# mikkleini/slam.net

Measured on AMD Instinct MI355X. Metric: candidate-pose distance evals/sec on 2048^2 map, 1080-ray scan, 1/2/4/8 GPU, higher is better.
Workload: dtype f32 transform + u16 gather / integer sum

## Files before the change

slam.net_amd/csrc/distance.hip:

```cpp
#include "cs_internal.h"
#include "det_trig.h"
#include <stdlib.h>
#include <algorithm>

#define K1_THREADS 256

__device__ static inline void k1_coords(const float4 q, const float2 p, float &fx, float &fy)
{
    fx = q.x + q.z * p.x;  fx = fx - q.w * p.y;
    fy = q.y + q.w * p.x;  fy = fy + q.z * p.y;
}

template <bool SAFE>
__device__ static inline void k1_gather_global(const uint16_t *__restrict__ map, int S, const float4 q, const float2 p,
                                               uint32_t &sum, uint32_t &cnt)
{
    float fx, fy;
    k1_coords(q, p, fx, fy);
    int ix, iy;
    if (SAFE) { ix = sh_f2i(fx); iy = sh_f2i(fy); }
    else      { ix = (int)fx;    iy = (int)fy; }
    const bool ok = ((unsigned)ix < (unsigned)S) & ((unsigned)iy < (unsigned)S);
    uint32_t v = 0;
    if (ok) v = map[(size_t)iy * S + ix];
// ... 187 lines not shown
__device__ static inline unsigned k1_tile_addr(int ix, int iy, int pitch2, int kofs)
{
    unsigned t, a;
    asm("v_lshl_add_u32 %0, %1, 1, %2" : "=v"(t) : "v"(ix), "s"(kofs));
    asm("v_mad_u32_u24 %0, %1, %2, %3" : "=v"(a) : "v"(iy), "s"(pitch2), "v"(t));
    return a;
}
__device__ static inline float k1_den(int v) { return __uint_as_float(v < 0 ? (0x80000000u | (unsigned)(-v)) : (unsigned)v); }
__device__ static inline unsigned k1_tile_addr_d(float fx, float fy, float two_d, float pitch2_d, float c_d)
{
    const float g = fmaf(truncf(fy), pitch2_d, fmaf(truncf(fx), two_d, c_d));
    return __float_as_uint(g);
}
typedef __attribute__((address_space(3))) const uint16_t k1_lds_u16;
__device__ static inline uint32_t k1_lds_load(unsigned addr) { return *(k1_lds_u16 *)(size_t)addr; }
typedef __attribute__((address_space(3))) const float k1_lds_f;
__device__ static inline float2 k1_point_lds(unsigned lds_addr)
{
    k1_lds_f *p = (k1_lds_f *)(size_t)lds_addr;
    return make_float2(p[0], p[1]);
}

typedef float k1_f32x4a8 __attribute__((ext_vector_type(4), aligned(8)));
__device__ static inline float4 k1_points2_lds(unsigned lds_addr)
{
    const k1_f32x4a8 v = *(__attribute__((address_space(3))) const k1_f32x4a8 *)(size_t)lds_addr;
    return make_float4(v.x, v.y, v.z, v.w);
}

__device__ static inline void k1_ray_box(const float *b, const float2 p, int &x0, int &y0, int &x1, int &y1)
{
    const float cx0 = b[4] * p.x, cx1 = b[5] * p.x, sy0 = b[6] * p.y, sy1 = b[7] * p.y;
    const float sx0 = b[6] * p.x, sx1 = b[7] * p.x, cy0 = b[4] * p.y, cy1 = b[5] * p.y;
    float xlo = b[0] + fminf(cx0, cx1);  xlo = xlo - fmaxf(sy0, sy1);
    float xhi = b[1] + fmaxf(cx0, cx1);  xhi = xhi - fminf(sy0, sy1);
    float ylo = b[2] + fminf(sx0, sx1);  ylo = ylo + fminf(cy0, cy1);
    float yhi = b[3] + fmaxf(sx0, sx1);  yhi = yhi + fmaxf(cy0, cy1);
    x0 = (int)xlo; x1 = (int)xhi; y0 = (int)ylo; y1 = (int)yhi;
}

__device__ static inline int k1_div(int a, int b)
{
    int q = (int)((float)a * __builtin_amdgcn_rcpf((float)b));
    const int r = a - q * b;
    if (r < 0) q--; else if (r >= b) q++;
    return q;
}

template <int CTRL, int ROWS> __device__ static inline int k1_dpp(int v) { return __builtin_amdgcn_update_dpp(v, v, CTRL, ROWS, 0xf, false); }
template <bool MAX> __device__ static inline int k1_wave_red(int x)
{
#define K1_MM(a, b) (MAX ? max(a, b) : min(a, b))
    x = K1_MM(x, (k1_dpp<0xB1, 0xf>(x)));
    x = K1_MM(x, (k1_dpp<0x4E, 0xf>(x)));
    x = K1_MM(x, (k1_dpp<0x124, 0xf>(x)));
    x = K1_MM(x, (k1_dpp<0x128, 0xf>(x)));
    x = K1_MM(x, (k1_dpp<0x142, 0xa>(x)));
    x = K1_MM(x, (k1_dpp<0x143, 0xc>(x)));
#undef K1_MM
    return x;
}
template <bool MAX> __device__ static inline float k1_wave_redf(float x)
{
#define K1_MM(a, b) (MAX ? fmaxf(a, b) : fminf(a, b))
    x = K1_MM(x, __int_as_float(k1_dpp<0xB1, 0xf>(__float_as_int(x))));
    x = K1_MM(x, __int_as_float(k1_dpp<0x4E, 0xf>(__float_as_int(x))));
    x = K1_MM(x, __int_as_float(k1_dpp<0x124, 0xf>(__float_as_int(x))));
    x = K1_MM(x, __int_as_float(k1_dpp<0x128, 0xf>(__float_as_int(x))));
    x = K1_MM(x, __int_as_float(k1_dpp<0x142, 0xa>(__float_as_int(x))));
    x = K1_MM(x, __int_as_float(k1_dpp<0x143, 0xc>(__float_as_int(x))));
#undef K1_MM
    return x;
}

struct k1_wg_t { int g, nc, nbp, bp, rlo, rhi, chunk; };
__device__ __forceinline__ k1_wg_t k1_wg_decode(const k1_args &a, const int bid)
{
    int g, chunk, nc, nbp = 1;
    if ((int)bid < a.n_tab_wgs) {
        const unsigned pw = ((const unsigned *)a.wg_pos)[bid >> 2];
        const int p = (int)((pw >> ((bid & 3u) * 8u)) & 0xffu);
        const k1_args::tab_rec rec = a.tab[p];
        nc = rec.nc;
        chunk = bid - (int)rec.first;
        g = rec.group;
        nbp = rec.nbp;
    } else {
        const int b = bid - a.n_tab_wgs;
        nc = a.uni_nc;
        chunk = b / (unsigned)a.uni_ng;
        g = a.uni_g0 + (b - chunk * a.uni_ng);
    }
    const int rc = chunk / nbp, bp = chunk - rc * nbp, nrc = nc / nbp;
    int rlo, rhi;
#define K1_CUT(i) ((int)((((const unsigned *)a.cut)[(i) >> 1] >> (((i) & 1) * 16)) & 0xffffu))
    if (a.uni_cut && (int)bid >= a.n_tab_wgs) {
        rlo = K1_CUT(chunk); rhi = K1_CUT(chunk + 1);
    } else if (a.tab_cut && (int)bid < a.n_tab_wgs) {
        const int i0 = a.tab_cut + (int)bid;
        rlo = K1_CUT(i0);
        rhi = rc + 1 < nrc ? K1_CUT(i0 + nbp) : a.n_rays;
    } else
#undef K1_CUT
    if (a.n_rays <= 46340) {
        rlo = (int)(((unsigned)rc * (unsigned)a.n_rays) / (unsigned)nrc); rhi = (int)(((unsigned)(rc + 1) * (unsigned)a.n_rays) / (unsigned)nrc);
    } else { rlo = (int)(((long long)rc * a.n_rays) / nrc); rhi = (int)(((long long)(rc + 1) * a.n_rays) / nrc); }
    k1_wg_t W; W.g = g; W.nc = nc; W.nbp = nbp; W.bp = bp; W.rlo = rlo; W.rhi = rhi; W.chunk = chunk;
    return W;
}

__device__ __forceinline__ void k1_bounds_from_jitter(const k1_args &a, const float gb[6], float *bnd, const int lane)
{
    const float scale = a.scale;
    const float pxl = (a.bx + gb[0]) * scale + 0.5f, pxh = (a.bx + gb[1]) * scale + 0.5f;
    const float pyl = (a.by + gb[2]) * scale + 0.5f, pyh = (a.by + gb[3]) * scale + 0.5f;
    const float tlf = a.bth + gb[4], thf = a.bth + gb[5];
    const double n2 = rint((double)tlf * 0.15915494309189535) * 6.283185307179586;
    const float rl = (float)((double)tlf - n2), rh = (float)((double)thf - n2);
    const float as = scale, pad = as * 1.0e-4f;
    const float cl = __cosf(rl) * as, ch = __cosf(rh) * as, sl = __sinf(rl) * as, sh = __sinf(rh) * as;
    float clo = fminf(cl, ch) - pad, chi = fmaxf(cl, ch) + pad, slo = fminf(sl, sh) - pad, shi = fmaxf(sl, sh) + pad;
    const bool all = !(rh - rl < 6.2f);
    {
        const int k_lo = (int)ceilf((rl - 1.0e-3f) * 0.636619772f), span = (int)floorf((rh + 1.0e-3f) * 0.636619772f) - k_lo;
        if (all || ((0 - k_lo) & 3) <= span) chi = as + pad;
        if (all || ((1 - k_lo) & 3) <= span) shi = as + pad;
        if (all || ((2 - k_lo) & 3) <= span) clo = -as - pad;
        if (all || ((3 - k_lo) & 3) <= span) slo = -as - pad;
    }
    const float4 qlo = make_float4(pxl, pyl, 0.f, 0.f), qhi = make_float4(pxh, pyh, 0.f, 0.f);
    if (lane == 0) {
        *(float4 *)&bnd[0] = make_float4(qlo.x, qhi.x, qlo.y, qhi.y);
        *(float4 *)&bnd[4] = make_float4(clo, chi, slo, shi);
    }
}

#ifndef K1_DMA0
#define K1_DMA0 0
#endif
#ifndef K1_EXP
#define K1_EXP 0
#endif
typedef unsigned int k1_u32x4 __attribute__((ext_vector_type(4)));

#ifndef K1_VGPR_CAP
#define K1_VGPR_CAP __attribute__((amdgpu_num_vgpr(104)))
#endif
template <int MODE, bool VERIFY, int CPL, int GROUP, bool LAT = false>
__global__ void __launch_bounds__(GROUP / CPL, GROUP / CPL / 64 / 2) K1_VGPR_CAP
k1_search_tiled(const k1_args a)
{
    constexpr int LANES = GROUP / CPL, NW = LANES / 64, PF = 65536 / (LANES * 16);
    constexpr int RU = (K1_MAXR + LANES - 1) / LANES;
    extern __shared__ __attribute__((aligned(16))) char smem[];
    const unsigned smem_lds = (unsigned)(size_t)(__attribute__((address_space(3))) char *)smem;
    __shared__ __attribute__((aligned(16))) int stepbuf[K1_MAXSTEPS * 8];
    __shared__ __attribute__((aligned(16))) float2 cpts[K1_MAXR + 4];
    __shared__ int2 pieces[K1_MAXP];
    __shared__ __attribute__((aligned(16))) float wred[NW][8];
    __shared__ __attribute__((aligned(16))) float bnd[8];
    __shared__ unsigned long long wkey[NW];
    __shared__ unsigned wfin[NW];
    __shared__ int s_nsteps;
    __shared__ int s_plan_ok;
    const unsigned cpts_lds = (unsigned)(size_t)(__attribute__((address_space(3))) char *)cpts;

    const uint16_t *__restrict__ map = a.map;
    const int S = a.S, count = a.count;
    const int t = threadIdx.x, lane = t & 63;
    int zv;
    asm volatile("v_mov_b32 %0, 0" : "=v"(zv));
    const int wv = __builtin_amdgcn_readfirstlane(t >> 6);
    const k1_wg_t W = k1_wg_decode(a, (int)blockIdx.x);
    const int g = W.g, nc = W.nc, nbp = W.nbp;
    if (a.ring_reset && blockIdx.x == 0 && t == 0)
        __hip_atomic_store(a.ring_reset, ~0ull, __ATOMIC_RELAXED, __HIP_MEMORY_SCOPE_AGENT);
    if (a.started && blockIdx.x == 0 && t == 0)
        __hip_atomic_store(a.started, a.launch_no, __ATOMIC_RELAXED, __HIP_MEMORY_SCOPE_SYSTEM);
    K1_STAMP(0)
#ifdef K1_TIMES
    if (t == 0 && blockIdx.x < 4096) { for (int k = 0; k < 8; k++) g_k1_sub[blockIdx.x * 8 + k] = 0; }
    if (t == 0 && blockIdx.x < 4096) { for (int k = 10; k < 16; k++) g_k1_times[blockIdx.x * 16 + k] = 0; g_k1_times[blockIdx.x * 16 + 14] = (unsigned long long)g; g_k1_times[blockIdx.x * 16 + 15] = (unsigned long long)nc; }
    if (lane == 0 && blockIdx.x < 4096) g_k1_wstart[blockIdx.x * 16 + (wv & 15)] = wall_clock64();
    if (t == 0 && blockIdx.x < 4096) {
        unsigned hw, xcc;
        asm volatile("s_getreg_b32 %0, hwreg(HW_REG_HW_ID)" : "=s"(hw));
        asm volatile("s_getreg_b32 %0, hwreg(HW_REG_XCC_ID)" : "=s"(xcc));
        g_k1_wstart[blockIdx.x * 16 + 15] = ((unsigned long long)(xcc & 15u) << 16) | ((hw >> 8) & 0xffu);
    }
#endif
    const int bp = W.bp, rlo = W.rlo, rhi = W.rhi;
    const int nrays = rhi - rlo;
    if (a.scan_flag) {
        uint32_t v = 0;
        if (wv == 0) {
            int spins = 0;
            for (;;) {
                v = __hip_atomic_load(a.scan_flag, __ATOMIC_RELAXED, __HIP_MEMORY_SCOPE_SYSTEM);
                if ((v & 0x7fffffffu) == a.scan_seq) break;
                if (++spins > (1 << 23)) { if (t == 0) atomicAdd(a.verify, 1u); v = 0x80000000u; break; }
                __builtin_amdgcn_s_sleep(32);
            }
            if (blockIdx.x == 0 && t == 0) { ((uint32_t *)a.scan_flag)[8] = (uint32_t)spins; ((uint32_t *)a.scan_flag)[9] += (uint32_t)spins; }
            if (lane == 0) s_plan_ok = (int)v;
        }
        __syncthreads();
        v = (uint32_t)s_plan_ok;
        __syncthreads();
        if (__builtin_amdgcn_readfirstlane(v) & 0x80000000u) return;
    }
    const int blk_first = a.ray_blk[rlo + zv].z;
    const int blk_last_v = a.ray_blk[rhi - 1 + zv].z;

    const bool pre = MODE == 1 && a.grp_bounds != nullptr;
    float gb[6];
    if (pre) {
#pragma unroll
        for (int k = 0; k < 6; k++) gb[k] = a.grp_bounds[8 * (size_t)g + k];
    }
    const bool planned = MODE == 1 && !LAT && pre && a.plan_rec != nullptr;
    uint2 prw = make_uint2(0u, 0u);
    if (planned && wv == 0) prw = a.plan_rec[(size_t)blockIdx.x * (K1_PLAN_REC_WORDS / 2) + lane];
    float4 q[CPL];
    float c3[CPL][3];
#pragma unroll
    for (int k = 0; k < CPL; k++) {
        const int j = g * GROUP + k * LANES + t;
        const int jc = j < count ? j : count - 1;
        if (MODE == 0) q[k] = a.pxcs[jc];
        else { c3[k][0] = a.src3[3 * jc]; c3[k][1] = a.src3[3 * jc + 1]; c3[k][2] = a.src3[3 * jc + 2]; }
    }
    int4 rinfo[RU];
    float2 rpt[RU];
#pragma unroll
    for (int u = 0; u < RU; u++) {
        const int i = u * LANES + t;
        const int r = rlo + (i < nrays ? i : 0);
        rinfo[u] = make_int4(0, 0, 0, 0); rpt[u] = make_float2(0.f, 0.f);
        if (i < nrays) { rinfo[u] = a.ray_blk[r]; rpt[u] = a.pts[r]; }
    }
    if (t == 0) { s_nsteps = 0; s_plan_ok = 0; *(unsigned *)(smem + K1_ZERO_OFS) = 0u; }
    if (MODE != 0 && !pre) {
#pragma unroll
        for (int k = 0; k < CPL; k++) q[k] = k1_candidate<MODE == 0 ? 1 : MODE, true>(c3[k], a.bx, a.by, a.bth, a.scale);
    }
#pragma unroll
    for (int u = 0; u < RU; u++) {
        const int i = u * LANES + t;
        if (i < nrays) {
            cpts[i] = rpt[u];
            if (i == 0 || rinfo[u].x == rlo + i)
                pieces[rinfo[u].z - blk_first] = make_int2(i, (rinfo[u].y < rhi ? rinfo[u].y : rhi) - (rlo + i));
        }
    }
    bool have_plan = false;
    if (planned) {
        if (wv == 0) {
            const bool okl = ((lane & 3) != 3 || prw.y == a.plan_seq) && (lane != 0 || prw.x == a.plan_seq);
            const int ns = __builtin_amdgcn_readfirstlane((int)prw.y);
            const bool ok = __builtin_amdgcn_ballot_w64(okl) == ~0ull && ns >= 0 && ns <= K1_PLAN_STEPS;
            if (lane >= 4) *(int2 *)&stepbuf[2 * lane - 8] = make_int2((int)prw.x, (int)prw.y);
            if (lane == 0 && ok) { s_plan_ok = 1; s_nsteps = ns; }
        }
        __syncthreads();
        have_plan = __builtin_amdgcn_readfirstlane(s_plan_ok) != 0;
        if (VERIFY && t == 0) atomicAdd(a.verify + (have_plan ? 5 : 6), 1u);
    }
    K1_STAMP(1)
    if (!have_plan) {
    if (pre) {
        if (wv == 0) {
            k1_bounds_from_jitter(a, gb, bnd, lane);
        }
        __syncthreads();
        K1_STAMP(2)
    } else
    {
        float lo[4] = { q[0].x, q[0].y, q[0].z, q[0].w }, hi[4] = { q[0].x, q[0].y, q[0].z, q[0].w };
#pragma unroll
        for (int k = 1; k < CPL; k++) {
            lo[0] = fminf(lo[0], q[k].x); hi[0] = fmaxf(hi[0], q[k].x); lo[1] = fminf(lo[1], q[k].y); hi[1] = fmaxf(hi[1], q[k].y);
            lo[2] = fminf(lo[2], q[k].z); hi[2] = fmaxf(hi[2], q[k].z); lo[3] = fminf(lo[3], q[k].w); hi[3] = fmaxf(hi[3], q[k].w);
        }
        const float m0 = k1_wave_redf<false>(lo[0]), m1 = k1_wave_redf<true>(hi[0]);
        const float m2 = k1_wave_redf<false>(lo[1]), m3 = k1_wave_redf<true>(hi[1]);
        const float m4 = k1_wave_redf<false>(lo[2]), m5 = k1_wave_redf<true>(hi[2]);
        const float m6 = k1_wave_redf<false>(lo[3]), m7 = k1_wave_redf<true>(hi[3]);
        if (lane == 63) {
            *(float4 *)&wred[wv][0] = make_float4(m0, m1, m2, m3);
            *(float4 *)&wred[wv][4] = make_float4(m4, m5, m6, m7);
        }
        __syncthreads();
        K1_STAMP(2)
        if (t < 8) {
            float v[NW];
#pragma unroll
            for (int w = 0; w < NW; w++) v[w] = wred[w][t];
            float x = v[0];
#pragma unroll
            for (int w = 1; w < NW; w++) x = (t & 1) ? fmaxf(x, v[w]) : fminf(x, v[w]);
            bnd[t] = x;
        }
        __syncthreads();
    }
    K1_STAMP(3)
    const int npieces = __builtin_amdgcn_readfirstlane(blk_last_v - blk_first + 1);
#define K1_PIECE_STAMP K1_STAMP(4)
#define K1_STEP_SLOT(i) (i)
#define K1_PIECE_RAY(i) (i)
#include "k1_pieces.inc"
#undef K1_PIECE_RAY
#undef K1_STEP_SLOT
#undef K1_PIECE_STAMP
    __syncthreads();
    }
#ifdef K1_TIMES
    else if (t == 0 && blockIdx.x < 4096) { const unsigned long long now_ = wall_clock64(); for (int k = 2; k <= 4; k++) g_k1_times[blockIdx.x * 16 + k] = now_; }
#endif
    const int nsteps = s_nsteps;
    K1_STAMP(5)

    uint32_t sum[CPL], cnt[CPL];
#pragma unroll
    for (int k = 0; k < CPL; k++) { sum[k] = 0; cnt[k] = 0; }
    if (LAT && !(MODE != 0 && a.grp_bounds != nullptr)) {
#pragma unroll
        for (int k = 1; k < CPL; k++)
            if (g * GROUP + k * LANES + t < count && (__float_as_uint(q[k].z) != __float_as_uint(q[0].z) || __float_as_uint(q[k].w) != __float_as_uint(q[0].w)))
                atomicAdd(a.verify, 1u);
    }
    uint32_t cnt_all = 0;
    if (nsteps > 0) {
        k1_u32x4 R[PF];
        int dst[PF];
#define K1_PREFETCH(step, enable)                                                                   \
        {                                                                                           \
             \
             \
             \
            const int4 pa_ = *(const int4 *)&stepbuf[(step) * 8];                                   \
            const int shift_ = __builtin_amdgcn_readfirstlane(stepbuf[(step) * 8 + 4]);             \
            const int w8_ = __builtin_amdgcn_readfirstlane(pa_.z), h_ = (enable) ? __builtin_amdgcn_readfirstlane(pa_.w) : 0; \
            const int rpi = 64 >> shift_;                          \
            const int srow = lane >> shift_, scol = lane & ((1 << shift_) - 1);                     \
            const bool colok = scol < (w8_ >> 3);                                                   \
            const int cc = colok ? scol : 0;                                                        \
            const unsigned S2_ = (unsigned)S * 2u;                                                  \
            const unsigned gofs = ((unsigned)__builtin_amdgcn_readfirstlane(pa_.y) * (unsigned)S + (unsigned)__builtin_amdgcn_readfirstlane(pa_.x)) * 2u; \
            const int pitchb = w8_ << 1;                                                            \
            const int row0 = wv * rpi + srow, rstep = NW * rpi;                                     \
            unsigned vofs = gofs + (unsigned)row0 * S2_ + ((unsigned)cc << 4);                      \
            int ldsd = K1_TILE_OFS + (cc << 4) + row0 * pitchb;                                     \
            const unsigned vstep = (unsigned)rstep * S2_;                                           \
            const int lstep = rstep * pitchb;                                                       \
            _Pragma("unroll") for (int k_ = 0; k_ < PF; k_++) {                                     \
                const bool live = colok & (row0 + k_ * rstep < h_);                                 \
                if (live && K1_EXP != 3) R[k_] = *(const k1_u32x4 *)((const char *)map + vofs);    \
                dst[k_] = live ? ldsd : -1;                                                         \
                vofs += vstep; ldsd += lstep;                                                       \
            }                                                                                       \
        }
#if K1_DMA0
        {
            const int4 pa_ = *(const int4 *)&stepbuf[0];
            const int w8_ = __builtin_amdgcn_readfirstlane(pa_.z), h_ = __builtin_amdgcn_readfirstlane(pa_.w);
            const int ncols = w8_ >> 3, nunits = ncols * h_;
            const unsigned S2_ = (unsigned)S * 2u;
            const unsigned gofs = ((unsigned)__builtin_amdgcn_readfirstlane(pa_.y) * (unsigned)S + (unsigned)__builtin_amdgcn_readfirstlane(pa_.x)) * 2u;
            const float rn = 1.0f / (float)ncols;
#pragma unroll
            for (int k_ = 0; k_ < PF; k_++) {
                const int e0 = (k_ * NW + wv) * 64;
                if (e0 < nunits && K1_EXP != 3) {
                    const int e = e0 + lane;
                    const int row = (int)(((float)e + 0.5f) * rn);
                    const int col = e - row * ncols;
                    if (e < nunits)
                        __builtin_amdgcn_global_load_lds((const __attribute__((address_space(1))) void *)((const char *)map + (gofs + (unsigned)row * S2_ + ((unsigned)col << 4))),
                                                         (__attribute__((address_space(3))) void *)(smem + K1_TILE_OFS + (e0 << 4)), 16, 0, 0);
                }
            }
#pragma unroll
            for (int k_ = 0; k_ < PF; k_++) dst[k_] = -1;
        }
#else
        K1_PREFETCH(0, true)
#endif
        if (MODE != 0 && pre) {
            {
#pragma unroll
            for (int k = 0; k < CPL; k++) { if (K1_EXP == 1) q[k] = make_float4(a.bx * a.scale + c3[k][0], a.by * a.scale + c3[k][1], a.scale, c3[k][2]); else q[k] = k1_candidate<MODE == 0 ? 1 : MODE, true>(c3[k], a.bx, a.by, a.bth, a.scale); }
            }
            if (LAT) {
#pragma unroll
                for (int k = 1; k < CPL; k++)
                    if (g * GROUP + k * LANES + t < count && (__float_as_uint(q[k].z) != __float_as_uint(q[0].z) || __float_as_uint(q[k].w) != __float_as_uint(q[0].w)))
                        atomicAdd(a.verify, 1u);
            }
        }
#ifdef K1_TIMES
        const unsigned long long sclk0 = clock64();
#endif
        for (int s = 0; s < nsteps; s++) {
#ifdef K1_TIMES
            const unsigned long long ts0 = wall_clock64();
#endif
            if (K1_DMA0 && s == 0) asm volatile("s_waitcnt vmcnt(0)" ::: "memory");
            else {
            __syncthreads();
#pragma unroll
            for (int k = 0; k < PF; k++) asm volatile("" : "+v"(R[k]));
#pragma unroll
            for (int k = 0; k < PF; k++) if (dst[k] >= 0 && K1_EXP != 3) *(k1_u32x4 *)(smem + dst[k]) = R[k];
            }
            __syncthreads();
            if (s == 0) K1_STAMP(6)
#ifdef K1_TIMES
            const unsigned long long ts1 = wall_clock64();
            if (s > 0) K1_SUB(0, ts1 - ts0)
#endif
            const int4 ca = *(const int4 *)&stepbuf[s * 8], cb = *(const int4 *)&stepbuf[s * 8 + 4];
            {
                const int sn = s + 1 < nsteps ? s + 1 : s;
                K1_PREFETCH(sn, s + 1 < nsteps)
            }
#ifdef K1_TIMES
            const unsigned long long ts2 = wall_clock64();
            K1_SUB(1, ts2 - ts1) K1_SUB(3, 1ull)
#endif
            const int kind = __builtin_amdgcn_readfirstlane(cb.y);
            const int nr = __builtin_amdgcn_readfirstlane(cb.z) >> 16;
#ifdef K1_TIMES
            if (t == 0 && blockIdx.x < 4096) g_k1_times[blockIdx.x * 16 + 10 + kind] += (unsigned long long)nr;
            if (t == 0 && blockIdx.x < 4096 && s < 3)
                g_k1_sub[blockIdx.x * 8 + 5 + s] = (unsigned long long)kind | ((unsigned long long)__builtin_amdgcn_readfirstlane(ca.z) << 4) | ((unsigned long long)__builtin_amdgcn_readfirstlane(ca.w) << 16) | ((unsigned long long)nr << 32);
#endif
            const unsigned pbase = cpts_lds + (unsigned)zv + (unsigned)(__builtin_amdgcn_readfirstlane(cb.z) & 0xffff) * 8u;
            const int x0a = __builtin_amdgcn_readfirstlane(ca.x), y0 = __builtin_amdgcn_readfirstlane(ca.y);
            const int w8 = __builtin_amdgcn_readfirstlane(ca.z), h = __builtin_amdgcn_readfirstlane(ca.w);
            const int pitch2 = w8 << 1;
            const int kofs = (int)smem_lds + K1_TILE_OFS - ((y0 * w8 + x0a) << 1);
            const unsigned zaddr = smem_lds + K1_ZERO_OFS + (unsigned)zv;
            const bool daddr = !a.noden && (unsigned)S * (unsigned)pitch2 + 2u * (unsigned)S + (1u << 18) < (1u << 23);
            float two_v, p2d_v, cd_v;
            {
                const float two_s = k1_den(2), p2d_s = k1_den(pitch2), cd_s = k1_den(kofs);
                asm volatile("v_mov_b32 %0, %1" : "=v"(two_v) : "s"(two_s));
                asm volatile("v_mov_b32 %0, %1" : "=v"(p2d_v) : "s"(p2d_s));
                asm volatile("v_mov_b32 %0, %1" : "=v"(cd_v) : "s"(cd_s));
            }
            if (K1_EXP == 2 || K1_EXP == 3) { sum[0] += (uint32_t)nr; continue; }
            if (kind != K1_KIND_GLOBAL) {
                const bool checked = kind == K1_KIND_BAND;
                uint32_t va[CPL], vb[CPL];
                int r = 0;
                float4 pn = k1_points2_lds(pbase);
                float2 pa_n = make_float2(pn.x, pn.y), pb_n = make_float2(pn.z, pn.w);
#pragma unroll
                for (int k = 0; k < CPL; k++) { va[k] = k1_lds_load(zaddr); vb[k] = k1_lds_load(zaddr); }
                __builtin_amdgcn_sched_barrier(0);
                if (!checked && daddr) {
#define K1_DPAIR(P, NEXTREAD)                                                                       \
                    {                                                                               \
                        unsigned ada[CPL], adb[CPL];                                                \
                        float cxa_ = 0.f, sya_ = 0.f, sxa_ = 0.f, cya_ = 0.f, cxb_ = 0.f, syb_ = 0.f, sxb_ = 0.f, cyb_ = 0.f; \
                        if (LAT) {                                                                  \
                            cxa_ = q[0].z * (P).x; sya_ = q[0].w * (P).y; sxa_ = q[0].w * (P).x; cya_ = q[0].z * (P).y; \
                            cxb_ = q[0].z * (P).z; syb_ = q[0].w * (P).w; sxb_ = q[0].w * (P).z; cyb_ = q[0].z * (P).w; \
                        }                                                                           \
                        _Pragma("unroll") for (int k = 0; k < CPL; k++) {                           \
                            float fxa, fya, fxb, fyb;                                               \
                            if (LAT) {                                                              \
                                fxa = q[k].x + cxa_; fxa = fxa - sya_; fya = q[k].y + sxa_; fya = fya + cya_; \
                                fxb = q[k].x + cxb_; fxb = fxb - syb_; fyb = q[k].y + sxb_; fyb = fyb + cyb_; \
                            } else {                                                                \
                                k1_coords(q[k], make_float2((P).x, (P).y), fxa, fya);               \
                                k1_coords(q[k], make_float2((P).z, (P).w), fxb, fyb);               \
                            }                                                                       \
                            ada[k] = k1_tile_addr_d(fxa, fya, two_v, p2d_v, cd_v);                  \
                            adb[k] = k1_tile_addr_d(fxb, fyb, two_v, p2d_v, cd_v);                  \
                            if (VERIFY) {                                                           \
                                const int ixa = (int)fxa, iya = (int)fya, ixb = (int)fxb, iyb = (int)fyb; \
                                if (ixa < x0a || ixa >= x0a + w8 || iya < y0 || iya >= y0 + h ||    \
                                    ixb < x0a || ixb >= x0a + w8 || iyb < y0 || iyb >= y0 + h) atomicAdd(a.verify, 1u); \
                                else if (ada[k] != k1_tile_addr(ixa, iya, pitch2, kofs) || adb[k] != k1_tile_addr(ixb, iyb, pitch2, kofs) || \
                                         map[(size_t)iya * S + ixa] != *(const uint16_t *)(smem + (ada[k] - smem_lds)) || \
                                         map[(size_t)iyb * S + ixb] != *(const uint16_t *)(smem + (adb[k] - smem_lds))) \
                                    atomicAdd(a.verify, 1u);                \
                            }                                                                       \
                        }                                                                           \
                        __builtin_amdgcn_sched_barrier(0);                                          \
                        NEXTREAD;      \
                        _Pragma("unroll") for (int k = 0; k < CPL; k++) sum[k] += va[k] + vb[k];    \
                        _Pragma("unroll") for (int k = 0; k < CPL; k++) { va[k] = k1_lds_load(ada[k]); vb[k] = k1_lds_load(adb[k]); } \
                        __builtin_amdgcn_sched_barrier(0);                                          \
                    }
                    for (; r + 3 < nr; r += 4) {
                        const float4 p0 = pn;
                        float4 p1;
                        K1_DPAIR(p0, p1 = k1_points2_lds(pbase + r * 8 + 16))
                        K1_DPAIR(p1, pn = k1_points2_lds(pbase + r * 8 + 32))
                    }
                    if (r + 1 < nr) {
                        const float4 p0 = pn;
                        K1_DPAIR(p0, pn = k1_points2_lds(pbase + r * 8 + 16))
                        r += 2;
                    }
#undef K1_DPAIR
                    pa_n = make_float2(pn.x, pn.y);
                    cnt_all += (uint32_t)nr;
                } else if (!checked) {
                    for (; r + 1 < nr; r += 2) {
                        const float2 pa = pa_n, pb = pb_n;
                        pa_n = k1_point_lds(pbase + r * 8 + 16); pb_n = k1_point_lds(pbase + r * 8 + 24);
                        unsigned ada[CPL], adb[CPL];
#pragma unroll
                        for (int k = 0; k < CPL; k++) {
                            float fxa, fya, fxb, fyb;
                            k1_coords(q[k], pa, fxa, fya);
                            k1_coords(q[k], pb, fxb, fyb);
                            const int ixa = (int)fxa, iya = (int)fya, ixb = (int)fxb, iyb = (int)fyb;
                            ada[k] = k1_tile_addr(ixa, iya, pitch2, kofs);
                            adb[k] = k1_tile_addr(ixb, iyb, pitch2, kofs);
                            if (VERIFY) {
                                if (ixa < x0a || ixa >= x0a + w8 || iya < y0 || iya >= y0 + h ||
                                    ixb < x0a || ixb >= x0a + w8 || iyb < y0 || iyb >= y0 + h) atomicAdd(a.verify, 1u);
                                else if (map[(size_t)iya * S + ixa] != *(const uint16_t *)(smem + (ada[k] - smem_lds)) ||
                                         map[(size_t)iyb * S + ixb] != *(const uint16_t *)(smem + (adb[k] - smem_lds)))
                                    atomicAdd(a.verify, 1u);
                            }
                        }
                        __builtin_amdgcn_sched_barrier(0);
#pragma unroll
                        for (int k = 0; k < CPL; k++) sum[k] += va[k] + vb[k];
#pragma unroll
                        for (int k = 0; k < CPL; k++) { va[k] = k1_lds_load(ada[k]); vb[k] = k1_lds_load(adb[k]); }
                        __builtin_amdgcn_sched_barrier(0);
                    }
                    cnt_all += (uint32_t)nr;
                } else {
                    for (; r + 1 < nr; r += 2) {
                        const float2 pa = pa_n, pb = pb_n;
                        pa_n = k1_point_lds(pbase + r * 8 + 16); pb_n = k1_point_lds(pbase + r * 8 + 24);
                        unsigned ada[CPL], adb[CPL];
#pragma unroll
                        for (int k = 0; k < CPL; k++) {
                            float fxa, fya, fxb, fyb;
                            k1_coords(q[k], pa, fxa, fya);
                            k1_coords(q[k], pb, fxb, fyb);
                            const int ixa = (int)fxa, iya = (int)fya, ixb = (int)fxb, iyb = (int)fyb;
                            const bool oka = ((unsigned)(ixa - x0a) < (unsigned)w8) & ((unsigned)(iya - y0) < (unsigned)h);
                            const bool okb = ((unsigned)(ixb - x0a) < (unsigned)w8) & ((unsigned)(iyb - y0) < (unsigned)h);
                            const unsigned ta = k1_tile_addr(ixa, iya, pitch2, kofs), tb = k1_tile_addr(ixb, iyb, pitch2, kofs);
                            if (VERIFY) {
                                if (oka && map[(size_t)iya * S + ixa] != *(const uint16_t *)(smem + (ta - smem_lds))) atomicAdd(a.verify, 1u);
                                if (okb && map[(size_t)iyb * S + ixb] != *(const uint16_t *)(smem + (tb - smem_lds))) atomicAdd(a.verify, 1u);
                            }
                            ada[k] = oka ? ta : zaddr;
                            adb[k] = okb ? tb : zaddr;
                            cnt[k] += (oka ? 1u : 0u) + (okb ? 1u : 0u);
                        }
                        __builtin_amdgcn_sched_barrier(0);
#pragma unroll
                        for (int k = 0; k < CPL; k++) sum[k] += va[k] + vb[k];
#pragma unroll
                        for (int k = 0; k < CPL; k++) { va[k] = k1_lds_load(ada[k]); vb[k] = k1_lds_load(adb[k]); }
                        __builtin_amdgcn_sched_barrier(0);
                    }
                }
                if (r < nr) {
                    const float2 pa = pa_n;
#pragma unroll
                    for (int k = 0; k < CPL; k++) {
                        float fx, fy;
                        k1_coords(q[k], pa, fx, fy);
                        const int ix = (int)fx, iy = (int)fy;
                        const bool ok = ((unsigned)(ix - x0a) < (unsigned)w8) & ((unsigned)(iy - y0) < (unsigned)h);
                        if (VERIFY) {
                            if (!ok && !checked) atomicAdd(a.verify, 1u);
                            if (ok && map[(size_t)iy * S + ix] != *(const uint16_t *)(smem + (k1_tile_addr(ix, iy, pitch2, kofs) - smem_lds))) atomicAdd(a.verify, 1u);
                        }
                        sum[k] += k1_lds_load(ok ? k1_tile_addr(ix, iy, pitch2, kofs) : zaddr);
                        if (checked) cnt[k] += ok ? 1u : 0u;
                    }
                }
#pragma unroll
                for (int k = 0; k < CPL; k++) sum[k] += va[k] + vb[k];
                if (VERIFY && t == 0) atomicAdd(a.verify + (checked ? 4 : 1), (unsigned)(nr * 4));
            } else {
                int r = 0;
                for (; r + 1 < nr; r += 2) {
                    const float2 pa = k1_point_lds(pbase + r * 8), pb = k1_point_lds(pbase + r * 8 + 8);
                    uint32_t ga[CPL], gb[CPL]; bool oka[CPL], okb[CPL];
#pragma unroll
                    for (int k = 0; k < CPL; k++) {
                        float fxa, fya, fxb, fyb;
                        k1_coords(q[k], pa, fxa, fya);
                        k1_coords(q[k], pb, fxb, fyb);
                        const int ixa = (int)fxa, iya = (int)fya, ixb = (int)fxb, iyb = (int)fyb;
                        oka[k] = ((unsigned)ixa < (unsigned)S) & ((unsigned)iya < (unsigned)S);
                        okb[k] = ((unsigned)ixb < (unsigned)S) & ((unsigned)iyb < (unsigned)S);
                        ga[k] = map[oka[k] ? (size_t)iya * S + ixa : 0];
                        gb[k] = map[okb[k] ? (size_t)iyb * S + ixb : 0];
                    }
#pragma unroll
                    for (int k = 0; k < CPL; k++) {
                        sum[k] += (oka[k] ? ga[k] : 0u) + (okb[k] ? gb[k] : 0u);
                        cnt[k] += (oka[k] ? 1u : 0u) + (okb[k] ? 1u : 0u);
                    }
                }
                if (r < nr) {
                    const float2 pa = k1_point_lds(pbase + r * 8);
#pragma unroll
                    for (int k = 0; k < CPL; k++) k1_gather_global<false>(map, S, q[k], pa, sum[k], cnt[k]);
                }
                if (VERIFY && t == 0) atomicAdd(a.verify + 3, (unsigned)(nr * 4));
            }
#ifdef K1_TIMES
            K1_SUB(2, wall_clock64() - ts2)
#endif
        }
#ifdef K1_TIMES
        K1_SUB(4, clock64() - sclk0)
#endif
#undef K1_PREFETCH
    }
    K1_STAMP(7)

    typedef unsigned long long u64;
    if (K1_EXP == 4) { if (sum[0] == 0x12345u && cnt[0] == 77u) a.verify[0] = 1u; return; }
    u64 *acc = a.acc + (size_t)g * GROUP + (size_t)t;
    u64 tot[CPL];
#pragma unroll
    for (int k = 0; k < CPL; k++) {
        const u64 add = (u64)sum[k] | ((u64)((cnt[k] | cnt_all) ? 1u : 0u) << K1_ACC_INMAP) | (1ull << K1_ACC_ARRIVED);
        tot[k] = __hip_atomic_fetch_add(acc + k * LANES, add, __ATOMIC_RELAXED, __HIP_MEMORY_SCOPE_AGENT) + add;
    }
    u64 key = ~0ull;
    unsigned nfin = 0;
#pragma unroll
    for (int k = 0; k < CPL; k++) {
        if ((unsigned)(tot[k] >> K1_ACC_ARRIVED) == (unsigned)nc) {
            __hip_atomic_store(acc + k * LANES, 0ull, __ATOMIC_RELAXED, __HIP_MEMORY_SCOPE_AGENT);
            const int j = g * GROUP + k * LANES + t;
            if (j < count) {
                const u64 kk = k1_finish(tot[k] & ((1ull << K1_ACC_INMAP) - 1), (uint32_t)(tot[k] >> K1_ACC_INMAP) & ((1u << (K1_ACC_ARRIVED - K1_ACC_INMAP)) - 1u),
                                         a.n_rays, a.ev_idx ? a.ev_idx[j] : j, a.dist_out);
                key = kk < key ? kk : key;
                nfin++;
            }
        }
    }
    K1_STAMP(8)
    if (__builtin_amdgcn_ballot_w64(nfin != 0) != 0) {
        for (int off = 32; off > 0; off >>= 1) {
            const u64 o = __shfl_down(key, off, 64);
            key = o < key ? o : key;
            nfin += (unsigned)__shfl_down((int)nfin, off, 64);
        }
    }
    if (a.ring_slot) {
        if (lane == 0 && nfin != 0) (void)__hip_atomic_fetch_min(a.ring_slot, key, __ATOMIC_RELAXED, __HIP_MEMORY_SCOPE_AGENT);
        K1_STAMP(9)
        return;
    }
    if (lane == 0) { wkey[wv] = key; wfin[wv] = nfin; }
    __syncthreads();
    if (t != 0) return;
    for (int w = 1; w < NW; w++) { key = wkey[w] < key ? wkey[w] : key; nfin += wfin[w]; }
    if (nfin == 0) return;
    (void)__hip_atomic_fetch_min(a.gmin, key, __ATOMIC_RELAXED, __HIP_MEMORY_SCOPE_AGENT);
    asm volatile("s_waitcnt vmcnt(0)" ::: "memory");
    const unsigned before = __hip_atomic_fetch_add(a.done, nfin, __ATOMIC_RELAXED, __HIP_MEMORY_SCOPE_AGENT);
    if (before + nfin != (unsigned)count) return;
    const u64 best = __hip_atomic_load(a.gmin, __ATOMIC_RELAXED, __HIP_MEMORY_SCOPE_AGENT);
    __hip_atomic_store(a.gmin, ~0ull, __ATOMIC_RELAXED, __HIP_MEMORY_SCOPE_AGENT);
    __hip_atomic_store(a.done, 0u, __ATOMIC_RELAXED, __HIP_MEMORY_SCOPE_AGENT);
    __hip_atomic_store(a.key_out, best, __ATOMIC_RELAXED, __HIP_MEMORY_SCOPE_AGENT);
    if (a.sig) asm volatile("s_waitcnt vmcnt(0)" ::: "memory");
    float bx = 0.0f, by = 0.0f, bthn = 0.0f;
    if (a.best_pose) {
        const uint32_t flat = (uint32_t)best;
        float th = a.bth;
        bx = a.bx; by = a.by;
        if (flat > 0) { bx = a.bx + a.offs_flat[3 * (flat - 1)]; by = a.by + a.offs_flat[3 * (flat - 1) + 1]; th = a.bth + a.offs_flat[3 * (flat - 1) + 2]; }
        bthn = sh_normalize_angle(th);
        a.best_pose[0] = bx; a.best_pose[1] = by; a.best_pose[2] = bthn;
        a.best_pose[3] = th;
    }
    if (a.sig) __hip_atomic_store(a.sig, a.sig_val, __ATOMIC_RELAXED, __HIP_MEMORY_SCOPE_SYSTEM);
    if (a.done_flag) {
        *(unsigned long long *)(a.done_flag - 15) = best;
        if (a.best_pose) { float *mp = (float *)(a.done_flag - 13); mp[0] = bx; mp[1] = by; mp[2] = bthn; }
        __hip_atomic_store(a.done_flag, a.done_val, __ATOMIC_RELEASE, __HIP_MEMORY_SCOPE_SYSTEM);
    }
    K1_STAMP(9)
}


__device__ static inline int k1_plan_slot(const int i) { return i <= K1_PLAN_STEPS ? i : K1_PLAN_STEPS + 1; }
template <int GROUP, int CPL>
__global__ void __launch_bounds__(64)
k1_plan(const k1_args a, const int n_wgs)
{
    constexpr int NW = 1, PF = 64;
    const int lane = threadIdx.x, wv = 0;
    const uint32_t seq = a.plan_seq;
    if ((int)blockIdx.x >= n_wgs) return;
    __shared__ __attribute__((aligned(16))) int stepbuf[(K1_PLAN_STEPS + 2) * 8];
    __shared__ int2 pieces[K1_MAXP];
    __shared__ __attribute__((aligned(16))) float bnd[8];
    __shared__ int s_nsteps;
    const int S = a.S;
    const k1_wg_t W = k1_wg_decode(a, (int)blockIdx.x);
    const int g = W.g, nbp = W.nbp, bp = W.bp, rlo = W.rlo, rhi = W.rhi, nrays = rhi - rlo;
    float gb[6];
#pragma unroll
    for (int k = 0; k < 6; k++) gb[k] = a.grp_bounds[8 * (size_t)g + k];
    const int blk_first = a.ray_blk[rlo].z, blk_last = a.ray_blk[rhi - 1].z;
    if (lane == 0) s_nsteps = 0;
    for (int i = lane; i < nrays; i += 64) {
        const int4 ri = a.ray_blk[rlo + i];
        const int pidx = ri.z - blk_first;
        if ((i == 0 || ri.x == rlo + i) && (unsigned)pidx < (unsigned)K1_MAXP) pieces[pidx] = make_int2(i, (ri.y < rhi ? ri.y : rhi) - (rlo + i));
    }
    const float2 *cpts = a.pts + rlo;
    k1_bounds_from_jitter(a, gb, bnd, lane);
    __syncthreads();
    const int npieces = min(blk_last - blk_first + 1, K1_MAXP);
#define K1_PIECE_STAMP
#define K1_STEP_SLOT(i) k1_plan_slot(i)
#define K1_PIECE_RAY(i) min(max((i), 0), nrays - 1)
#include "k1_pieces.inc"
#undef K1_PIECE_RAY
#undef K1_STEP_SLOT
#undef K1_PIECE_STAMP
    __syncthreads();
    const int nsteps = s_nsteps;
    const bool fits = nsteps <= K1_PLAN_STEPS;
    const int unit = lane >> 2, wp = lane & 3;
    uint2 w = make_uint2(0u, 0u);
    if (unit > 0 && fits && unit - 1 < nsteps) { w.x = (uint32_t)stepbuf[(unit - 1) * 8 + 2 * wp]; w.y = (uint32_t)stepbuf[(unit - 1) * 8 + 2 * wp + 1]; }
    if (lane == 0) { w.x = seq; w.y = (uint32_t)(fits ? nsteps : -1); }
    if (wp == 3) w.y = seq;
    __hip_atomic_store((unsigned long long *)(a.plan_rec + (size_t)blockIdx.x * (K1_PLAN_REC_WORDS / 2) + lane), ((unsigned long long)w.y << 32) | w.x,
                       __ATOMIC_RELAXED, __HIP_MEMORY_SCOPE_AGENT);
}

int32_t cs_plan_drain(slamhip_cs *cs)
{
    if (cs->plan_stream) SH_HIP(hipStreamSynchronize(cs->plan_stream));
    return SLAMHIP_OK;
}

void cs_plan_free(slamhip_cs *cs)
{
    if (cs->plan_stream) (void)hipStreamSynchronize(cs->plan_stream);
    for (int i = 0; i < K1_PLAN_SLOTS; i++) {
        (void)hipFree(cs->d_plan_rec[i]);
        cs->d_plan_rec[i] = nullptr; cs->plan_slot_user[i] = 0;
    }
    cs->plan_cap_wgs = 0;
}

int32_t cs_alloc_candidates(slamhip_cs *cs, int count)
{
    if (count <= cs->cap_cand) return SLAMHIP_OK;
    SH_TRY(cs_plan_drain(cs));
// ... 1021 lines not shown
```

Baseline: 1.083 billion.

## Cut staging registers, pipeline odd tail, use float-denormal addressing for global gather

The tile-staging prefetch now keeps a live-row count plus a base LDS address instead of a per-slot destination array. Strides become shifts based on the log2 wavefront count, which frees VGPRs under the 104-register cap. The odd trailing ray in the unchecked LDS path now goes through the same software-pipelined load pattern as the paired loop. The global-memory fallback gets a denormal-float address computation (truncf and fma) as an alternative to integer multiply when S<=2048. This adds macro complexity and relies on exact denormal float arithmetic to form addresses.

```diff
diff --git a/slam.net_amd/csrc/distance.hip b/slam.net_amd/csrc/distance.hip
--- a/slam.net_amd/csrc/distance.hip
+++ b/slam.net_amd/csrc/distance.hip
@@ -363,6 +363,8 @@
 {
     constexpr int LANES = GROUP / CPL, NW = LANES / 64, PF = 65536 / (LANES * 16);
     constexpr int RU = (K1_MAXR + LANES - 1) / LANES;
+    constexpr int LGNW = NW == 4 ? 2 : NW == 8 ? 3 : NW == 16 ? 4 : -1;
+    static_assert(LGNW >= 0, "the staging strides are shifts: 4, 8 or 16 wavefronts per workgroup");
     extern __shared__ __attribute__((aligned(16))) char smem[];
     const unsigned smem_lds = (unsigned)(size_t)(__attribute__((address_space(3))) char *)smem;
     __shared__ __attribute__((aligned(16))) int stepbuf[K1_MAXSTEPS * 8];
@@ -543,7 +545,7 @@
     uint32_t cnt_all = 0;
     if (nsteps > 0) {
         k1_u32x4 R[PF];
-        int dst[PF];
+        int nlive = 0, ldsd0 = 0, lstep_s = 0;
 #define K1_PREFETCH(step, enable)                                                                   \
         {                                                                                           \
              \
@@ -553,22 +555,22 @@
             const int shift_ = __builtin_amdgcn_readfirstlane(stepbuf[(step) * 8 + 4]);             \
             const int w8_ = __builtin_amdgcn_readfirstlane(pa_.z), h_ = (enable) ? __builtin_amdgcn_readfirstlane(pa_.w) : 0; \
             const int rpi = 64 >> shift_;                          \
+            const int lgstep_ = LGNW + 6 - shift_;               \
             const int srow = lane >> shift_, scol = lane & ((1 << shift_) - 1);                     \
             const bool colok = scol < (w8_ >> 3);                                                   \
-            const int cc = colok ? scol : 0;                                                        \
             const unsigned S2_ = (unsigned)S * 2u;                                                  \
             const unsigned gofs = ((unsigned)__builtin_amdgcn_readfirstlane(pa_.y) * (unsigned)S + (unsigned)__builtin_amdgcn_readfirstlane(pa_.x)) * 2u; \
             const int pitchb = w8_ << 1;                                                            \
-            const int row0 = wv * rpi + srow, rstep = NW * rpi;                                     \
-            unsigned vofs = gofs + (unsigned)row0 * S2_ + ((unsigned)cc << 4);                      \
-            int ldsd = K1_TILE_OFS + (cc << 4) + row0 * pitchb;                                     \
-            const unsigned vstep = (unsigned)rstep * S2_;                                           \
-            const int lstep = rstep * pitchb;                                                       \
+            const int row0 = wv * rpi + srow;                                        \
+             \
+            unsigned vofs = gofs + __umul24((unsigned)row0, S2_) + ((unsigned)scol << 4);           \
+            ldsd0 = (int)smem_lds + K1_TILE_OFS + (scol << 4) + (int)__umul24((unsigned)row0, (unsigned)pitchb);    \
+            nlive = colok ? (h_ - row0 + (1 << lgstep_) - 1) >> lgstep_ : 0;     \
+            const unsigned vstep = S2_ << lgstep_;                                                  \
+            lstep_s = pitchb << lgstep_;                                                            \
             _Pragma("unroll") for (int k_ = 0; k_ < PF; k_++) {                                     \
-                const bool live = colok & (row0 + k_ * rstep < h_);                                 \
-                if (live && K1_EXP != 3) R[k_] = *(const k1_u32x4 *)((const char *)map + vofs);    \
-                dst[k_] = live ? ldsd : -1;                                                         \
-                vofs += vstep; ldsd += lstep;                                                       \
+                if (k_ < nlive && K1_EXP != 3) R[k_] = *(const k1_u32x4 *)((const char *)map + vofs);    \
+                vofs += vstep;                                                                      \
             }                                                                                       \
         }
 #if K1_DMA0
@@ -591,8 +593,7 @@
                                                          (__attribute__((address_space(3))) void *)(smem + K1_TILE_OFS + (e0 << 4)), 16, 0, 0);
                 }
             }
-#pragma unroll
-            for (int k_ = 0; k_ < PF; k_++) dst[k_] = -1;
+            nlive = 0;
         }
 #else
         K1_PREFETCH(0, true)
@@ -622,7 +623,7 @@
 #pragma unroll
             for (int k = 0; k < PF; k++) asm volatile("" : "+v"(R[k]));
 #pragma unroll
-            for (int k = 0; k < PF; k++) if (dst[k] >= 0 && K1_EXP != 3) *(k1_u32x4 *)(smem + dst[k]) = R[k];
+            for (int k = 0; k < PF; k++) { if (k < nlive && K1_EXP != 3) *(__attribute__((address_space(3))) k1_u32x4 *)(size_t)(unsigned)ldsd0 = R[k]; ldsd0 += lstep_s; }
             }
             __syncthreads();
             if (s == 0) K1_STAMP(6)
@@ -779,7 +780,29 @@
                         __builtin_amdgcn_sched_barrier(0);
                     }
                 }
-                if (r < nr) {
+                if ((nr & 1) && !checked) {
+                    const float2 pa = pa_n;
+                    unsigned ada[CPL];
+#pragma unroll
+                    for (int k = 0; k < CPL; k++) {
+                        float fx, fy;
+                        k1_coords(q[k], pa, fx, fy);
+                        if (daddr) ada[k] = k1_tile_addr_d(fx, fy, two_v, p2d_v, cd_v);
+                        else ada[k] = k1_tile_addr((int)fx, (int)fy, pitch2, kofs);
+                        if (VERIFY) {
+                            const int ix = (int)fx, iy = (int)fy;
+                            if (ix < x0a || ix >= x0a + w8 || iy < y0 || iy >= y0 + h) atomicAdd(a.verify, 1u);
+                            else if (ada[k] != k1_tile_addr(ix, iy, pitch2, kofs) ||
+                                     map[(size_t)iy * S + ix] != *(const uint16_t *)(smem + (ada[k] - smem_lds))) atomicAdd(a.verify, 1u);
+                        }
+                    }
+                    __builtin_amdgcn_sched_barrier(0);
+#pragma unroll
+                    for (int k = 0; k < CPL; k++) sum[k] += va[k] + vb[k];
+#pragma unroll
+                    for (int k = 0; k < CPL; k++) { va[k] = k1_lds_load(ada[k]); vb[k] = k1_lds_load(zaddr); }
+                    __builtin_amdgcn_sched_barrier(0);
+                } else if (nr & 1) {
                     const float2 pa = pa_n;
 #pragma unroll
                     for (int k = 0; k < CPL; k++) {
@@ -788,43 +811,78 @@
                         const int ix = (int)fx, iy = (int)fy;
                         const bool ok = ((unsigned)(ix - x0a) < (unsigned)w8) & ((unsigned)(iy - y0) < (unsigned)h);
                         if (VERIFY) {
-                            if (!ok && !checked) atomicAdd(a.verify, 1u);
                             if (ok && map[(size_t)iy * S + ix] != *(const uint16_t *)(smem + (k1_tile_addr(ix, iy, pitch2, kofs) - smem_lds))) atomicAdd(a.verify, 1u);
                         }
                         sum[k] += k1_lds_load(ok ? k1_tile_addr(ix, iy, pitch2, kofs) : zaddr);
-                        if (checked) cnt[k] += ok ? 1u : 0u;
+                        cnt[k] += ok ? 1u : 0u;
                     }
                 }
 #pragma unroll
                 for (int k = 0; k < CPL; k++) sum[k] += va[k] + vb[k];
                 if (VERIFY && t == 0) atomicAdd(a.verify + (checked ? 4 : 1), (unsigned)(nr * 4));
             } else {
-                int r = 0;
-                for (; r + 1 < nr; r += 2) {
-                    const float2 pa = k1_point_lds(pbase + r * 8), pb = k1_point_lds(pbase + r * 8 + 8);
-                    uint32_t ga[CPL], gb[CPL]; bool oka[CPL], okb[CPL];
-#pragma unroll
-                    for (int k = 0; k < CPL; k++) {
-                        float fxa, fya, fxb, fyb;
-                        k1_coords(q[k], pa, fxa, fya);
-                        k1_coords(q[k], pb, fxb, fyb);
-                        const int ixa = (int)fxa, iya = (int)fya, ixb = (int)fxb, iyb = (int)fyb;
-                        oka[k] = ((unsigned)ixa < (unsigned)S) & ((unsigned)iya < (unsigned)S);
-                        okb[k] = ((unsigned)ixb < (unsigned)S) & ((unsigned)iyb < (unsigned)S);
-                        ga[k] = map[oka[k] ? (size_t)iya * S + ixa : 0];
-                        gb[k] = map[okb[k] ? (size_t)iyb * S + ixb : 0];
-                    }
-#pragma unroll
-                    for (int k = 0; k < CPL; k++) {
-                        sum[k] += (oka[k] ? ga[k] : 0u) + (okb[k] ? gb[k] : 0u);
-                        cnt[k] += (oka[k] ? 1u : 0u) + (okb[k] ? 1u : 0u);
-                    }
+                const bool gden = !a.noden && (unsigned)S <= 2048u;
+                float s2d_v, lim_v, zero_v;
+                {
+                    const float s2d_s = k1_den(2 * S), lim_s = (float)S, zero_s = 0.0f;
+                    asm volatile("v_mov_b32 %0, %1" : "=v"(s2d_v) : "s"(s2d_s));
+                    asm volatile("v_mov_b32 %0, %1" : "=v"(lim_v) : "s"(lim_s));
+                    asm volatile("v_mov_b32 %0, %1" : "=v"(zero_v) : "s"(zero_s));
                 }
-                if (r < nr) {
-                    const float2 pa = k1_point_lds(pbase + r * 8);
-#pragma unroll
-                    for (int k = 0; k < CPL; k++) k1_gather_global<false>(map, S, q[k], pa, sum[k], cnt[k]);
+#define K1_GOFS(DEN, fx_, fy_, ofs_, ok_)                                                           \
+                {                                                                                   \
+                    if (DEN) {                                                                      \
+                        const float tx_ = truncf(fx_), ty_ = truncf(fy_);                           \
+                        ok_ = (fminf(tx_, ty_) >= zero_v) & (fmaxf(tx_, ty_) < lim_v);              \
+                        ofs_ = ok_ ? __float_as_uint(fmaf(ty_, s2d_v, fmaf(tx_, two_v, zero_v))) : 0u; \
+                    } else {                                                                        \
+                        const int ix_ = (int)(fx_), iy_ = (int)(fy_);                               \
+                        ok_ = ((unsigned)ix_ < (unsigned)S) & ((unsigned)iy_ < (unsigned)S);        \
+                        ofs_ = ok_ ? (__umul24((unsigned)iy_, (unsigned)S) + (unsigned)ix_) << 1 : 0u; \
+                    }                                                                               \
+                    asm("" : "+v"(ofs_));       \
+                    if (VERIFY) {                                                                   \
+                        const int ix_ = (int)(fx_), iy_ = (int)(fy_);                               \
+                        const bool in_ = ((unsigned)ix_ < (unsigned)S) & ((unsigned)iy_ < (unsigned)S); \
+                        if (in_ != ok_ || ofs_ != (in_ ? (unsigned)(((size_t)iy_ * S + ix_) * 2) : 0u)) atomicAdd(a.verify, 1u); \
+                    }                                                                               \
                 }
+#define K1_GLOOP(DEN)                                                                               \
+                {                                                                                   \
+                    for (int r = 0; r + 1 < nr; r += 2) {                                           \
+                        const float2 pa = k1_point_lds(pbase + r * 8), pb = k1_point_lds(pbase + r * 8 + 8); \
+                        uint32_t ga[CPL], gb[CPL]; bool oka[CPL], okb[CPL];                         \
+                        _Pragma("unroll") for (int k = 0; k < CPL; k++) {                           \
+                            float fxa, fya, fxb, fyb;                                               \
+                            k1_coords(q[k], pa, fxa, fya);                                          \
+                            k1_coords(q[k], pb, fxb, fyb);                                          \
+                            unsigned oa, ob;                                                        \
+                            K1_GOFS(DEN, fxa, fya, oa, oka[k])                                      \
+                            K1_GOFS(DEN, fxb, fyb, ob, okb[k])                                      \
+                            ga[k] = *(const uint16_t *)((const char *)map + oa);                    \
+                            gb[k] = *(const uint16_t *)((const char *)map + ob);                    \
+                        }                                                                           \
+                        _Pragma("unroll") for (int k = 0; k < CPL; k++) {                           \
+                            sum[k] += (oka[k] ? ga[k] : 0u) + (okb[k] ? gb[k] : 0u);                \
+                            cnt[k] += (oka[k] ? 1u : 0u) + (okb[k] ? 1u : 0u);                      \
+                        }                                                                           \
+                    }                                                                               \
+                    if (nr & 1) {                                                                   \
+                        const float2 pa = k1_point_lds(pbase + (nr - 1) * 8);                       \
+                        _Pragma("unroll") for (int k = 0; k < CPL; k++) {                           \
+                            float fx, fy;                                                           \
+                            k1_coords(q[k], pa, fx, fy);                                            \
+                            unsigned o; bool ok;                                                    \
+                            K1_GOFS(DEN, fx, fy, o, ok)                                             \
+                            const uint32_t v = *(const uint16_t *)((const char *)map + o);          \
+                            sum[k] += ok ? v : 0u;                                                  \
+                            cnt[k] += ok ? 1u : 0u;                                                 \
+                        }                                                                           \
+                    }                                                                               \
+                }
+                if (gden) K1_GLOOP(true) else K1_GLOOP(false)
+#undef K1_GLOOP
+#undef K1_GOFS
                 if (VERIFY && t == 0) atomicAdd(a.verify + 3, (unsigned)(nr * 4));
             }
 #ifdef K1_TIMES
```

Result: slower. 1.050 billion (-3.1%).
